# trvon/yams

Hardware: AMD Instinct MI355X
Metric: k-NN QPS + recall@k, 100M x 768 fp32 cosine top-100; ingest GB/s SHA-256+CDC (higher is better)
Workload: dtype i8 (MFMA filter, exact i32 accumulate) + f64 (exact re-score)

## Files before the change

yams_amd/csrc/scan_api.cpp:

```cpp
#include <chrono>
#include <algorithm>
#include <cmath>
#include <cstdio>
#include <cstdlib>
#include <cstring>
#include <vector>

#include "accel_ctx.h"
#include "scan_launch.h"

using namespace yams_accel;

namespace {

constexpr uint64_t kMfmaMinRows = 4096;
constexpr uint64_t kExactKeyBudget = 1ull << 31;
constexpr size_t kStatWords = 16;

uint32_t round_up(uint32_t v, uint32_t m) { return (v + m - 1) / m * m; }

ScanPlan make_plan(uint64_t n_rows, uint32_t dim, uint32_t nq, uint32_t k, bool bf16, int passes, bool l2_band, int depth = 0) {
    ScanPlan p;
    p.n_rows = n_rows; p.dim = dim; p.n_queries = nq;
    p.tile_rows = bf16 ? 256 : kTileRows;
// ... 457 lines not shown

yams_status_t run_filter(Batch& b, Filter& f, bool* done) {
    yams_accel_ctx* ctx = b.ctx; const yams_scan_corpus_t* corpus = b.io.corpus; hipStream_t st = b.st;
    const uint32_t nq = b.nq; const bool i8 = f.i8, bf16 = f.bf16;
    ScanLaunch& L = f.L; const ScanPlan& plan = L.plan;
    if (i8) L.dense = nullptr;
    else YA_TRY(ws_get(ctx, "dense", static_cast<size_t>(nq) * plan.sample_rows * 4, (void**)&L.dense));
    YA_TRY(ws_get(ctx, "gmax", static_cast<size_t>(nq) * plan.n_groups * 4, (void**)&L.gmax));
    YA_TRY(ws_get(ctx, "tau", static_cast<size_t>(nq) * 4, (void**)&f.d_tau));
    YA_TRY(ws_get(ctx, "list", static_cast<size_t>(nq) * plan.list_cap * 8, (void**)&f.d_list));
    const uint32_t gchunks = (plan.n_groups + kSelectCap - 1) / kSelectCap;
    YA_TRY(ws_get(ctx, "work32", static_cast<size_t>(2) * nq * std::max(1u, gchunks) * plan.tau_rank * 4, (void**)&f.d_work32));
    const uint32_t lchunks = (plan.list_cap + kSelectCap - 1) / kSelectCap, keep_max = kRescoreMax + 1;
    YA_TRY(ws_get(ctx, "work64", static_cast<size_t>(2) * nq * lchunks * keep_max * 8, (void**)&f.d_work64));
    L.tau = f.d_tau; L.tau_out = f.d_tau; L.list_count = b.d_lcount; L.list = f.d_list;
    if (i8) {
        L.i8_q_form = i8_takes_q_form(L, f.bf16_version);
        if (corpus->row_mask && corpus->row_mask_count) L.i8_mask_inflation = static_cast<double>(corpus->n_rows) / static_cast<double>(corpus->row_mask_count);
        const uint64_t regions = i8_log_regions(L);
        L.log_cap = i8_log_capacity(L);
        YA_TRY(ws_get(ctx, "i8_log_key", static_cast<size_t>(regions) * L.log_cap * i8_log_entry_bytes(L), (void**)&L.log_key));
        YA_TRY(ws_get(ctx, "i8_log_q", static_cast<size_t>(regions) * L.log_cap * 4, (void**)&L.log_q));
        const uint64_t sync_words = i8_sync_words(L);
        const size_t z_cnt = (static_cast<size_t>(regions) * 4 + 255) & ~size_t(255), z_over = (static_cast<size_t>(nq) * 4 + 255) & ~size_t(255);
        unsigned char* zeroed;
        YA_TRY(ws_get(ctx, "i8_zeroed", z_cnt + z_over + static_cast<size_t>(sync_words) * 4, (void**)&zeroed));
        XcdDealPrep deal{};
        uint64_t deal_words = 0;
        if (i8_xcd_deal_plan(L, &deal, &deal_words)) {
            YA_TRY(ws_get(ctx, "i8_xcd", static_cast<size_t>(deal_words) * 4, (void**)&L.i8_xcd));
// ... 19 lines not shown
                }
                k.forced = 1;
            }
#endif
        }
        YA_HIP(ctx, launch_prep_i8(st, b.d_qprep, nq, L.q_pad, b.dim, const_cast<int8_t*>(L.q_i8), const_cast<float*>(L.q_meta), L.i8_l2,
                                   reinterpret_cast<uint32_t*>(zeroed), (z_cnt + z_over) / 4 + sync_words, (corpus->i8_flags & YAMS_SCAN_I8_ROTATED) != 0, &deal));
        L.log_cnt = reinterpret_cast<uint32_t*>(zeroed);
        L.q_over = f.d_qover = reinterpret_cast<uint32_t*>(zeroed + z_cnt);
        if (sync_words) L.i8_sync = reinterpret_cast<uint32_t*>(zeroed + z_cnt + z_over);
    }
    { TimedRegion tr(ctx, "scan_sample");
      if (i8) YA_HIP(ctx, launch_scan_i8(st, L, 0, f.bf16_version));
      else if (bf16) YA_HIP(ctx, launch_scan_bf16(st, L, b.metric, 0, f.passes, f.bf16_version)); else YA_HIP(ctx, launch_scan_sample(st, L, b.metric));
      tr.end(); }
    if (b.retry) YA_HIP(ctx, hipMemcpyAsync(f.d_tau, b.retry->forced_tau, static_cast<size_t>(nq) * 4, hipMemcpyDeviceToDevice, st));
    else YA_HIP(ctx, launch_select_tau(st, L, f.d_work32));
    if (i8 && L.i8_l2) {
        YA_HIP(ctx, launch_i8_l2_thresholds(st, f.d_tau, L.q_meta, nq, L.q_pad, b.dim, b.d_l2_stats, const_cast<float*>(L.q_thr), const_cast<uint32_t*>(L.i8_q_bias)));
        YA_HIP(ctx, launch_i8_l2_rows(st, corpus->rows_nsq, corpus->rows_i8_meta, b.d_l2_nmin, corpus->n_rows, b.d_l2_stats, const_cast<float*>(L.i8_l2_meta),
                                      const_cast<uint8_t*>(L.i8_row_bias)));
    } else if (i8) YA_HIP(ctx, launch_i8_thresholds(st, f.d_tau, L.q_meta, nq, L.q_pad, const_cast<float*>(L.q_thr)));
    if (i8) YA_HIP(ctx, launch_i8_collect_sample(st, L)); else YA_HIP(ctx, launch_collect_sample(st, L));
    if (i8 && L.i8_l2) YA_HIP(ctx, launch_i8_l2_add_special(st, L, b.d_l2_special, b.l2_n_special));
    { GatedSweep gs(ctx, st);
      TimedRegion tr(ctx, "scan_filter");
      if (i8) YA_HIP(ctx, launch_scan_i8(st, L, 1, f.bf16_version));
      else if (bf16) YA_HIP(ctx, launch_scan_bf16(st, L, b.metric, 1, f.passes, f.bf16_version)); else YA_HIP(ctx, launch_scan_filter(st, L, b.metric));
      tr.end();
      gs.leave(); }
    if (i8) YA_HIP(ctx, launch_i8_log_gather(st, L));
#ifdef YAMS_ACCEL_MEASURE
    if (!(i8 && L.i8_sync)) {}
    else if (const char* dump = std::getenv("YAMS_ACCEL_DUMP_SYNC")) {
        std::vector<uint32_t> h(i8_sync_words(L));
        YA_HIP(ctx, hipMemcpyAsync(h.data(), L.i8_sync, h.size() * 4, hipMemcpyDeviceToHost, st));
        YA_HIP(ctx, hipStreamSynchronize(st));
// ... 458 lines not shown
```

yams_amd/csrc/scan_i8_kernel.hip:

```cpp
#include <climits>
#include <cstdlib>
#include <type_traits>

#include "lds_dma.h"
#include "scan_args.h"
#include "xcd_deal.h"

namespace yams_accel {

using i32x4v = __attribute__((ext_vector_type(4))) int;

constexpr int I8_ROWS = 256, I8_QUERIES = 256, I8_THREADS = 512;
constexpr int I8_SLAB = 64;
constexpr int I8_NST = 4;
constexpr int I8_A_BYTES = I8_ROWS * I8_SLAB;
constexpr int I8_B_BYTES = I8_QUERIES * I8_SLAB;
constexpr int I8_STAGE = I8_A_BYTES + I8_B_BYTES;
constexpr int I8_BLOCK_ROWS = 64;

__device__ __forceinline__ int i8_swz(int row) {
    const int j = (row >> 2) & 3;
    return (((j ^ (j >> 1)) & 1) << 1) | (j >> 1);
}

// ... 757 lines not shown
                asm volatile("s_waitcnt vmcnt(0)" ::: "memory");
                __builtin_amdgcn_sched_barrier(0);
            } else { qthr_wait(); thresholds(); }
            k_new = take_result();
            if (n_qt > 1 && more && pacing && pace_now) {
                asm volatile("" : "+v"(sib));
                uint32_t polls = 0;
                for (; polls < R_POLLS; ++polls) {
                    if (__builtin_amdgcn_ballot_w64(sib + R_WINDOW < k_new) == 0) break;
                    __builtin_amdgcn_s_sleep(8);
                    asm volatile("global_load_dword %0, %1, off sc0 sc1\n\ts_waitcnt vmcnt(0)" : "=v"(sib) : "v"(sync_sib) : "memory");
                }
                if (polls == R_POLLS) pacing = false;
            }
        } else if (SAMPLE) {
            asm volatile("s_waitcnt vmcnt(0)" ::: "memory");
            k_new = take_result();
            const uint32_t sel_c = 2u * u + (k_cur & 1u);
            if (sel_c < a.n_sel_tiles) {
                const float ninf = -__builtin_inff();
                const uint32_t gid = (sel_c * static_cast<uint32_t>(I8_ROWS) + static_cast<uint32_t>((wid & 3) * 64)) / 16u + static_cast<uint32_t>(lq);
#pragma unroll
                for (int cb = 0; cb < 8; ++cb) {
                    const uint32_t qi = q0 + static_cast<uint32_t>(cb * 16 + l15);
                    const float4 qm = reinterpret_cast<const float4*>(lds + R_ZS_THR)[cb * 16 + l15];
                    const float S = sb_cur * qm.x, K = fmaf(eb_cur, qm.y, qm.z);
                    float m = ninf;
#pragma unroll
                    for (int rb = 0; rb < 4; ++rb) {
                        const uint64_t rbase = strip + static_cast<uint32_t>(16 * rb + 4 * lq);
                        const uint32_t mw = a.row_mask ? mask_word(a.row_mask, rbase & ~31ull, a.n_rows) >> (rbase & 31u) : 0xfu;
#pragma unroll
                        for (int r = 0; r < 4; ++r) {
                            const float uu = fmaf(static_cast<float>(acc[rb][cb][r]), S, K);
                            m = fmaxf(m, (rbase + r < a.n_rows && ((mw >> r) & 1u)) ? uu : ninf);
                        }
                    }
                    if (qi < a.n_queries) a.gmax[static_cast<uint64_t>(qi) * a.n_groups + gid] = (m != m) ? 0xffffffffu : f2ord(m);
                }
            }
            sb = __uint_as_float(static_cast<uint32_t>(meta_n));
            eb = __uint_as_float(static_cast<uint32_t>(meta_n >> 32));
        } else {
            asm volatile("s_waitcnt vmcnt(0)" ::: "memory");
            k_new = take_result();
            int t = 0;
#pragma unroll
            for (int rb = 0; rb < 4; ++rb)
#pragma unroll
                for (int cb = 0; cb < 8; ++cb)
#pragma unroll
                    for (int r = 0; r < 4; ++r) t += acc[rb][cb][r];
            if (t == 123456789 && a.list_cap == 0xffffffffu) a.list_count[0] = 1;
// ... 108 lines not shown
        if (!i8_entry_score<L2>(keys[i], q, rows_meta, q_meta, q_thr, l2, row, u)) continue;
        const uint32_t pos = slot0[q - q0] + atomicAdd(&hist[q - q0], 1u);
        if (pos < list_cap) list[static_cast<uint64_t>(q) * list_cap + pos] = pack_key(u, row);
    }
}

#ifdef YAMS_ACCEL_MEASURE
#include "scan_i8q_gather.h"
#endif

__global__ __launch_bounds__(256) void i8_collect_sample_kernel(const uint32_t* gmax, uint32_t n_groups, uint32_t n_queries,
                                                                const int8_t* rows_i8, const float* rows_meta, const int8_t* q_i8,
                                                                const float* q_meta, uint32_t q_pad, uint32_t dim,
                                                                uint32_t stride, uint64_t n_rows, const uint32_t* row_mask,
                                                                const float* tau, uint32_t* list_count, uint64_t* list,
                                                                uint32_t list_cap, const float* l2_rows_nsq, float l2_eps) {
    const uint32_t q = blockIdx.y;
    const float t = tau[q];
    const uint32_t* gm = gmax + static_cast<uint64_t>(q) * n_groups;
    const uint32_t nchunk = dim / 16;
    const int lane = threadIdx.x & 63;
    const float4 qm = reinterpret_cast<const float4*>(q_meta)[q];
    const uint32_t wave0 = (blockIdx.x * blockDim.x + threadIdx.x) & ~63u, wstep = gridDim.x * blockDim.x;
    for (uint32_t g0 = wave0; g0 < n_groups; g0 += wstep) {
        const uint32_t gl = g0 + static_cast<uint32_t>(lane);
        const bool hot = gl < n_groups && !(ord2f(gm[gl]) < t);
        for (uint64_t hm = __builtin_amdgcn_ballot_w64(hot); hm; hm &= hm - 1) {
            const uint32_t g = g0 + static_cast<uint32_t>(__builtin_ctzll(hm));
            const int i = lane & 15;
            const uint64_t sidx = static_cast<uint64_t>(g >> 2) * 64 + 4 * (g & 3) + 16 * (i >> 2) + (i & 3);
            const uint64_t row = (sidx / I8_ROWS) * stride * I8_ROWS + (sidx % I8_ROWS);
            const bool ok = row < n_rows && (!row_mask || row_allowed(row_mask, row));
            const uint64_t rr = row < n_rows ? row : n_rows - 1;
            int dot = 0;
            for (uint32_t ch = static_cast<uint32_t>(lane >> 4); ch < nchunk; ch += 4) {
                const int4 xv = *reinterpret_cast<const int4*>(rows_i8 + i8_blocked_offset(rr, ch * 16, dim));
                const int4 qv = *reinterpret_cast<const int4*>(q_i8 + (static_cast<uint64_t>(ch >> 2) * q_pad + q) * 64 + (ch & 3u) * 16);
                dot = __builtin_amdgcn_sdot4(xv.x, qv.x, dot, false);
                dot = __builtin_amdgcn_sdot4(xv.y, qv.y, dot, false);
                dot = __builtin_amdgcn_sdot4(xv.z, qv.z, dot, false);
                dot = __builtin_amdgcn_sdot4(xv.w, qv.w, dot, false);
            }
            dot += __shfl_xor(dot, 16);
            dot += __shfl_xor(dot, 32);
            if (lane < 16 && ok) {
                const float2 bm = reinterpret_cast<const float2*>(rows_meta)[row / I8_BLOCK_ROWS];
                const float S = bm.x * qm.x, K = fmaf(bm.y, qm.y, qm.z);
                float u = fmaf(static_cast<float>(dot), S, K);
                bool unbounded = false;
                if (l2_rows_nsq) {
                    const float nsq = l2_rows_nsq[row];
                    unbounded = !norm_in_range(nsq);
                    u = i8_l2_bound(u, nsq, l2_eps);
                }
                if (!unbounded && !(u < t)) {
                    const uint32_t pos = atomicAdd(&list_count[q], 1u);
                    if (pos < list_cap) list[static_cast<uint64_t>(q) * list_cap + pos] = pack_key(u, static_cast<uint32_t>(row));
                }
            }
        }
    }
}

__device__ inline uint32_t rot_sign(uint32_t i, uint32_t salt) {
    uint32_t v = i * 2654435761u + salt * 0x9E3779B9u;
    v ^= v >> 15; v *= 2246822519u; v ^= v >> 13; v *= 3266489917u; v ^= v >> 16;
    return v << 31;
}
__device__ inline void wave_lds_fence() {
    __builtin_amdgcn_fence(__ATOMIC_ACQ_REL, "wavefront");
    __builtin_amdgcn_wave_barrier();
}
template <int EPL>
__device__ inline void wave_fwht(float* w, int lane, uint32_t g0, uint32_t sign_salt, float scale) {
    float v[EPL];
// ... 288 lines not shown
    if (threadIdx.x == 0) {
        const float fd = static_cast<float>(dim);
        const float up = 1.0f + (fd + 16.f) * 5.9604645e-8f;
        q_meta[4 * q + 0] = t;
        q_meta[4 * q + 1] = ok ? sqrtf(csum) * up : 0.f;
        const float unit = raw ? (rot_p ? (sqrtf(csum) + sqrtf(red[0])) * up * 1.00001f : sqrtf(csum) * up) : 1.0f;
        q_meta[4 * q + 2] = ok ? sqrtf(red[0]) * up + ((fd + 32.f) * 5.9604645e-8f + 1e-6f + (rot_p ? 1e-5f : 0.f)) * unit : 0.f;
        q_meta[4 * q + 3] = 0.f;
    }
}

__global__ void i8_query_thresholds_kernel(const float* tau, const float* q_meta, uint32_t nq, uint32_t q_pad, float* q_thr) {
    const uint32_t q = blockIdx.x * blockDim.x + threadIdx.x;
    if (q >= q_pad) return;
    float A = __builtin_inff(), B = 0.f;
    if (q < nq) {
        const float t = q_meta[4 * q], c = q_meta[4 * q + 1], f = q_meta[4 * q + 2], ta = tau[q];
        if (ta != ta) A = -__builtin_inff();
        else {
            A = (ta - f) / t;
            A -= fabsf(A) * 1.9073486e-6f;
        }
        B = (c / t) * (1.0f + 1.9073486e-6f);
    }
    q_thr[2 * q] = A;
    q_thr[2 * q + 1] = B;
}

constexpr int L2S_WAVES = 16;
constexpr uint32_t I8_L2_MAX_SPECIAL = 64;
__global__ __launch_bounds__(L2S_WAVES * 64) void i8_l2_norm_stats_kernel(const float* rows_nsq, const float* rows_meta, uint64_t n_rows,
                                                                         uint64_t n_blocks, float* nmin_out, uint32_t* stats,
                                                                         uint32_t* special) {
    __shared__ uint32_t red[L2S_WAVES][5];
    const int lane = threadIdx.x & 63, wid = threadIdx.x >> 6;
    float qlo = __builtin_inff(), qhi = 0.f, sp = 0.f, em = 0.f;
    constexpr int NB = 4;
    const uint64_t step = static_cast<uint64_t>(gridDim.x) * L2S_WAVES;
    for (uint64_t blk0 = static_cast<uint64_t>(blockIdx.x) * L2S_WAVES + wid; blk0 < n_blocks; blk0 += step * NB) {
// ... 278 lines not shown
bool i8_takes_q_form(const ScanLaunch&, int) { return false; }
uint32_t i8_log_entry_bytes(const ScanLaunch&) { return 8u; }
#endif

uint64_t i8_log_regions(const ScanLaunch& L) {
    const ResidentPlan r = i8_resident_plan(L);
    if (r.use && L.i8_q_form) return static_cast<uint64_t>(r.n_streams) * r.n_qt * 4u;
    if (r.use) return static_cast<uint64_t>(r.n_streams) * r.n_qt * 8u;
    return static_cast<uint64_t>((2u * L.plan.n_filter_tiles + 7) / 8) * L.plan.n_qtiles * 8u * 4u;
}

hipError_t launch_i8_collect_sample(hipStream_t st, const ScanLaunch& L) {
    if (L.plan.sample_rows == 0 || L.plan.n_groups == 0) return hipSuccess;
    uint32_t gx = (L.plan.n_groups + 255) / 256;
    if (gx > 64) gx = 64;
#ifdef YAMS_ACCEL_MEASURE
    if (const char* e = std::getenv("YAMS_ACCEL_COLLECT_GX")) { const uint32_t v = static_cast<uint32_t>(std::atoi(e)); if (v >= 1 && v < gx) gx = v; }
#endif
    hipLaunchKernelGGL(i8_collect_sample_kernel, dim3(gx, L.plan.n_queries), dim3(256), 0, st, L.gmax, L.plan.n_groups,
                       L.plan.n_queries, L.rows_i8, L.rows_i8_meta, L.q_i8, L.q_meta, L.q_pad, L.plan.dim, L.plan.sample_stride,
                       L.plan.n_rows, L.row_mask, L.tau, L.list_count, L.list, L.plan.list_cap,
                       L.i8_l2 ? L.rows_nsq : nullptr, L.l2_eps);
    return hipGetLastError();
}

bool i8_xcd_deal_plan(const ScanLaunch& L, XcdDealPrep* p, uint64_t* table_words) {
    const ResidentPlan r = i8_resident_plan(L);
    if (!r.use) return false;
    p->n_units_filter = r.n_units;
    p->n_units_sample = (L.plan.n_sample_tiles + 1u) / 2u;
    p->streams_x = r.n_streams / XCD_DEAL_XCDS;
    p->n_qt = r.n_qt;
    *table_words = XCD_TABLE_TICKS + static_cast<uint64_t>(r.n_streams) * r.n_qt * XCD_TICKS_PER_WG;
    return true;
}

uint64_t i8_sync_words(const ScanLaunch& L) {
// ... 181 lines not shown
```

yams_amd/csrc/scan_kernels.hip:

```cpp
#include <algorithm>

#include "common.h"
#include "scan_args.h"

namespace yams_accel {

using f32x16 = __attribute__((ext_vector_type(16))) float;

constexpr int LDP = kSlabK + 4;
constexpr int STAGE_FLOATS = (kTileRows + kTileQueries) * LDP;
constexpr int SCAN_THREADS = 256;


template <int MODE, int METRIC>
__global__ __launch_bounds__(SCAN_THREADS, 2) void scan_tiles_kernel(ScanArgs a) {
    __shared__ __attribute__((aligned(16))) float lds[2 * STAGE_FLOATS];

    const uint32_t bid = blockIdx.x;
    const uint32_t xcd = bid & 7u;
    const uint32_t w = bid >> 3;
    const uint32_t qt = w % a.n_qtiles;
    const uint32_t sel = (w / a.n_qtiles) * 8u + xcd;
    if (sel >= a.n_sel_tiles) return;
    uint32_t tile;
// ... 388 lines not shown
    K* dst = out + static_cast<uint64_t>(qslot) * out_stride + static_cast<uint64_t>(blockIdx.x) * keep;
    if (c0 >= n) {
        for (uint32_t i = threadIdx.x; i < keep; i += 256) dst[i] = K(0);
        return;
    }
    const uint64_t left = n - c0;
    const uint64_t end = left < static_cast<uint64_t>(CAP) ? n : c0 + CAP;
    if (left <= 256) topk_block_sorted<K, 1>(src, c0, end, dst, keep, s);
    else if (left <= 512) topk_block_sorted<K, 2>(src, c0, end, dst, keep, s);
    else if (left <= 1024) topk_block_sorted<K, 4>(src, c0, end, dst, keep, s);
    else if (left <= 2048) topk_block_sorted<K, 8>(src, c0, end, dst, keep, s);
    else topk_block_sorted<K, 16>(src, c0, end, dst, keep, s);
}

constexpr int TAU_LIST = 2048;
__global__ __launch_bounds__(256) void tau_select_kernel(const uint32_t* gmax, uint32_t n_groups,
                                                         uint32_t rank, float* tau, const float* rows_meta, uint64_t n_blocks,
                                                         const float* q_meta, uint32_t rank2, uint32_t max_groups, float e_scale) {
    __shared__ uint32_t hist[2048];
    __shared__ uint32_t s_prefix, s_rank, s_count, s_v1, s_v2, s_va;
    __shared__ float s_red[4];
    const uint32_t q = blockIdx.x;
    const uint32_t* keys = gmax + static_cast<uint64_t>(q) * n_groups;
    if (n_groups < rank) {
        if (threadIdx.x == 0) tau[q] = -__builtin_inff();
        return;
    }
    if (rank >= 1 && rank <= 256) {
        const float e_mine = rows_meta != nullptr && n_blocks ? rows_meta[2 * ((n_blocks - 1) * threadIdx.x / 255) + 1] : 0.f;
        uint32_t mine = 0;
        for (uint32_t i = threadIdx.x; i < n_groups; i += 256) { const uint32_t k = keys[i]; mine = k > mine ? k : mine; }
        hist[threadIdx.x] = mine;
        if (threadIdx.x == 0) { s_count = 0; s_v1 = 0; s_v2 = 0; s_va = 0; }
        __syncthreads();
        uint32_t above = 0, at_or_above = 0;
        for (int j = 0; j < 256; ++j) { const uint32_t o = hist[j]; above += o > mine; at_or_above += o >= mine; }
        if (above < rank && rank <= at_or_above) s_prefix = mine;
        __syncthreads();
        const uint32_t L = s_prefix;
        __syncthreads();
        bool overflow = false;
        if (mine >= L)
            for (uint32_t i = threadIdx.x; i < n_groups; i += 256) {
                const uint32_t k = keys[i];
                if (k >= L) {
                    const uint32_t pos = atomicAdd(&s_count, 1u);
                    if (pos < TAU_LIST) hist[pos] = k; else overflow = true;
                }
            }
        if (!__syncthreads_or(overflow)) {
            const uint32_t c = s_count;
            if (max_groups > n_groups / 64) max_groups = n_groups / 64;
            const bool aware = rows_meta != nullptr && rank2 >= 5 && rank2 < rank && max_groups >= rank2;
            const uint32_t rank_a = rank2 - 4;
            for (uint32_t i = threadIdx.x; i < c; i += 256) {
                const uint32_t k = hist[i];
                uint32_t gt = 0, ge = 0;
                for (uint32_t j = 0; j < c; ++j) { const uint32_t o = hist[j]; gt += o > k; ge += o >= k; }
                if (gt < rank && rank <= ge) {
                    if (aware) s_v1 = k; else tau[q] = k ? ord2f(k) : -__builtin_inff();
                }
                if (aware && gt < rank2 && rank2 <= ge) s_v2 = k;
                if (aware && gt < rank_a && rank_a <= ge) s_va = k;
            }
            if (!aware) return;
            float e = e_mine;
#pragma unroll
            for (int d = 32; d >= 1; d >>= 1) e = fmaxf(e, __shfl_xor(e, d));
            if ((threadIdx.x & 63) == 0) s_red[threadIdx.x >> 6] = e;
            __syncthreads();
            const uint32_t v1 = s_v1, v2 = s_v2, va = s_va;
            float t_out = v1 ? ord2f(v1) : -__builtin_inff();
            bool want = false;
            float tp = 0.f;
            if (v1 && v2 && va) {
                e = fmaxf(fmaxf(s_red[0], s_red[1]), fmaxf(s_red[2], s_red[3]));
                const float4 qm = reinterpret_cast<const float4*>(q_meta)[q];
                const float E = fmaf(e, qm.y, qm.z) * e_scale;
                tp = ord2f(v2) - 2.0f * E;
                want = ord2f(va) - t_out < E && tp < t_out;
            }
            if (want) {
                const uint32_t lb = __syncthreads_count(mine != 0 && !(ord2f(mine) < tp));
                uint32_t n_reach = 0xffffffffu;
                if (lb <= max_groups) {
                    uint32_t cnt = 0;
                    for (uint32_t i = threadIdx.x; i < n_groups; i += 256) { const uint32_t k = keys[i]; cnt += k != 0 && !(ord2f(k) < tp); }
#pragma unroll
                    for (int d = 32; d >= 1; d >>= 1) cnt += __shfl_xor(cnt, d);
                    __syncthreads();
                    if ((threadIdx.x & 63) == 0) s_red[threadIdx.x >> 6] = __uint_as_float(cnt);
                    __syncthreads();
                    n_reach = __float_as_uint(s_red[0]) + __float_as_uint(s_red[1]) + __float_as_uint(s_red[2]) + __float_as_uint(s_red[3]);
                }
                if (n_reach <= max_groups) t_out = tp;
            }
            if (threadIdx.x == 0) tau[q] = t_out;
            return;
        }
        __syncthreads();
    }
    if (threadIdx.x == 0) { s_prefix = 0; s_rank = rank; }
    const int shifts[3] = {21, 10, 0};
    const int widths[3] = {11, 11, 10};
    for (int p = 0; p < 3; ++p) {
        const int shift = shifts[p], bins = 1 << widths[p];
        for (int i = threadIdx.x; i < 2048; i += 256) hist[i] = 0;
        __syncthreads();
        const uint32_t prefix = s_prefix;
        const int hi_shift = shift + widths[p];
        for (uint32_t i = threadIdx.x; i < n_groups; i += 256) {
            const uint32_t k = keys[i];
// ... 15 lines not shown
            const uint32_t r = s_rank;
            if (r > excl && r <= incl) {
                uint32_t above = excl;
                for (int j = 0; j < per; ++j) {
                    const int b = bins - 1 - (lane * per + j);
                    const uint32_t c = hist[b];
                    if (r <= above + c) { s_prefix = (prefix << widths[p]) | static_cast<uint32_t>(b); s_rank = r - above; break; }
                    above += c;
                }
            }
        }
        __syncthreads();
    }
    if (threadIdx.x == 0) {
        const uint32_t key = s_prefix;
        tau[q] = key ? ord2f(key) : -__builtin_inff();
    }
}

__global__ __launch_bounds__(256) void collect_sample_kernel(const float* dense, const uint32_t* gmax,
                                                             uint32_t n_groups, uint32_t n_queries,
                                                             uint64_t sample_rows, uint32_t tile_rows,
                                                             uint32_t stride,
                                                             uint64_t n_rows, const float* tau,
                                                             uint32_t* list_count, uint64_t* list,
                                                             uint32_t list_cap, int layout16) {
    const uint32_t q = blockIdx.y;
    const float t = tau[q];
    const uint32_t* gm = gmax + static_cast<uint64_t>(q) * n_groups;
    for (uint32_t g = blockIdx.x * blockDim.x + threadIdx.x; g < n_groups; g += gridDim.x * blockDim.x) {
        const float m = ord2f(gm[g]);
// ... 715 lines not shown
        cur = dst; cur_counts = nullptr; cur_stride = dst_stride; cur_n = chunks * keep;
        cur_qmap = nullptr;
        count_clip = 0xffffffffu;
        which ^= 1;
        if (chunks == 1) break;
    }
    *result = cur;
    *result_stride = cur_stride;
    return hipSuccess;
}

hipError_t launch_select_tau(hipStream_t st, const ScanLaunch& L, uint32_t* ) {
    const uint32_t nq = L.plan.n_queries;
    if (nq == 0) return hipSuccess;
    hipLaunchKernelGGL(tau_select_kernel, dim3(nq), dim3(256), 0, st, L.gmax, L.plan.n_groups,
                       L.plan.tau_rank, L.tau_out, L.tau_rows_meta, L.tau_n_blocks, L.q_meta, L.tau_rank2, L.tau_max_groups, L.tau_e_scale);
    LAUNCH_CHECK();
    return hipSuccess;
}

hipError_t launch_collect_sample(hipStream_t st, const ScanLaunch& L) {
    if (L.plan.sample_rows == 0 || L.plan.n_groups == 0) return hipSuccess;
    uint32_t gx = (L.plan.n_groups + 255) / 256;
    if (gx > 256) gx = 256;
    hipLaunchKernelGGL(collect_sample_kernel, dim3(gx, L.plan.n_queries), dim3(256), 0, st, L.dense,
                       L.gmax, L.plan.n_groups, L.plan.n_queries, L.plan.sample_rows, L.plan.tile_rows,
                       L.plan.sample_stride, L.plan.n_rows, L.tau, L.list_count, L.list, L.plan.list_cap,
                       L.sample_layout);
    LAUNCH_CHECK();
    return hipSuccess;
}
// ... 297 lines not shown
```

yams_amd/csrc/scan_launch.h:

```cpp
#pragma once
#include "common.h"
#include "xcd_deal.h"

namespace yams_accel {

struct ScanLaunch {
    ScanPlan plan;
    const float* rows = nullptr;
    const uint16_t* rows_bf16 = nullptr;
    const float* rows_nsq = nullptr;
    const int8_t* rows_i8 = nullptr;
    const float* rows_i8_meta = nullptr;
    const int8_t* q_i8 = nullptr;
    const float* q_meta = nullptr;
    const float* q_thr = nullptr;
    uint64_t* log_key = nullptr; uint32_t* log_q = nullptr; uint32_t* log_cnt = nullptr; uint32_t log_cap = 0;
    uint32_t* q_over = nullptr;
    uint32_t* i8_sync = nullptr;
    uint32_t* i8_xcd = nullptr;
    bool i8_l2 = false;
    const float* i8_l2_meta = nullptr;
    const uint8_t* i8_row_bias = nullptr;
    const uint32_t* i8_q_bias = nullptr;
    float l2_eps = 0.f;
    bool i8_sample_small_grid = false;
    int i8_form = 0;
    bool i8_q_form = false;
    double i8_mask_inflation = 1.0;
    int sample_layout = 0;
    const uint32_t* row_mask = nullptr;
    const float* qprep = nullptr;
    const uint16_t* q_hi = nullptr;
    const uint16_t* q_lo = nullptr;
    uint32_t q_pad = 0;
    float* dense = nullptr;
    uint32_t* gmax = nullptr;
    const float* tau = nullptr;
    float* tau_out = nullptr;
    const float* tau_rows_meta = nullptr; uint64_t tau_n_blocks = 0; uint32_t tau_rank2 = 0, tau_max_groups = 0; float tau_e_scale = 1.0f;
    uint32_t* list_count = nullptr;
    uint64_t* list = nullptr;
    const float* qnorm_up = nullptr;
    float err_coef = 0.f;
};

struct RescoreLaunch {
    const float* rows; uint64_t n_rows; uint32_t dim;
    const float* queries; const double* qnorm;
    const uint32_t* tie_rank; const uint32_t* rank_row; int64_t row_base;
    uint32_t stripe_rows, n_stripes, stripe_index;
    const uint64_t* cand; uint64_t cand_stride; uint32_t n_cand;
    const float* tau; const uint32_t* list_count; uint32_t list_cap; uint32_t all_rows_listed;
    const uint32_t* qmap; uint32_t n_slots;
    uint32_t k; float threshold; uint32_t flags; double err_bound;
// ... 116 lines not shown
```

Measured before the change: 16990.

## Chain tau select into thresholds and hot-group list; precompute sample group keys

The tau selection kernel now also writes the i8 query thresholds, which removes the separate threshold launch on the non-L2 path. It also records the indices of groups at or above tau in a small per-query hot list. The collect-sample kernel reads that list and scores only those groups, skipping the full gmax scan, and its grid is capped lower when the list is present. Separately, the sample-pass group max keys are computed before the vmcnt wait, using an integer-max fast path, so they overlap with outstanding loads. The cost is more LDS and branching in tau_select, plus a fallback to the full scan when the list overflows or a key is zero.

```diff
diff --git a/yams_amd/csrc/sample_chain.h b/yams_amd/csrc/sample_chain.h
--- /dev/null
+++ b/yams_amd/csrc/sample_chain.h
@@ -0,0 +1,39 @@
+#pragma once
+#include "contract_rules.h"
+
+namespace yams_accel {
+
+YAMS_RULE bool sample_max_int_ok(float S, float K) {
+    uint32_t sb, kb;
+    __builtin_memcpy(&sb, &S, 4);
+    __builtin_memcpy(&kb, &K, 4);
+    return sb < 0x7f800000u && (kb & 0x7fffffffu) < 0x7f800000u && kb != 0x80000000u;
+}
+
+YAMS_RULE uint32_t sample_group_key_int(int acc_max, bool any, float S, float K) {
+    return any ? f2ord(fmaf(static_cast<float>(acc_max), S, K)) : f2ord(-__builtin_inff());
+}
+
+YAMS_RULE uint32_t sample_group_key_rows(const int* acc, uint32_t live, float S, float K) {
+    float m = -__builtin_inff();
+    for (int l = 0; l < 16; ++l) {
+        const float uu = fmaf(static_cast<float>(acc[l]), S, K);
+        m = fmaxf(m, ((live >> l) & 1u) ? uu : -__builtin_inff());
+    }
+    return (m != m) ? 0xffffffffu : f2ord(m);
+}
+
+YAMS_RULE void i8_threshold_halves(float ta, float t, float c, float f, float& A, float& B) {
+    if (ta != ta) A = -__builtin_inff();
+    else {
+        A = (ta - f) / t;
+        A -= fabsf(A) * 1.9073486e-6f;
+    }
+    B = (c / t) * (1.0f + 1.9073486e-6f);
+}
+
+constexpr uint32_t HOT_STRIDE = 128, HOT_CAP = HOT_STRIDE - 1, HOT_SCAN = 0xffffffffu;
+
+YAMS_RULE bool hot_threshold_listable(float t) { return t == t && t != 0.0f; }
+
+}
diff --git a/yams_amd/csrc/scan_api.cpp b/yams_amd/csrc/scan_api.cpp
--- a/yams_amd/csrc/scan_api.cpp
+++ b/yams_amd/csrc/scan_api.cpp
@@ -7,6 +7,7 @@
 #include <vector>
 
 #include "accel_ctx.h"
+#include "sample_chain.h"
 #include "scan_launch.h"
 
 using namespace yams_accel;
@@ -495,6 +496,8 @@
     const uint32_t lchunks = (plan.list_cap + kSelectCap - 1) / kSelectCap, keep_max = kRescoreMax + 1;
     YA_TRY(ws_get(ctx, "work64", static_cast<size_t>(2) * nq * lchunks * keep_max * 8, (void**)&f.d_work64));
     L.tau = f.d_tau; L.tau_out = f.d_tau; L.list_count = b.d_lcount; L.list = f.d_list;
+    uint32_t* d_hot = nullptr;
+    if (i8) YA_TRY(ws_get(ctx, "i8_hot", static_cast<size_t>(nq) * HOT_STRIDE * 4, (void**)&d_hot));
     if (i8) {
         L.i8_q_form = i8_takes_q_form(L, f.bf16_version);
         if (corpus->row_mask && corpus->row_mask_count) L.i8_mask_inflation = static_cast<double>(corpus->n_rows) / static_cast<double>(corpus->row_mask_count);
@@ -544,13 +547,16 @@
       if (i8) YA_HIP(ctx, launch_scan_i8(st, L, 0, f.bf16_version));
       else if (bf16) YA_HIP(ctx, launch_scan_bf16(st, L, b.metric, 0, f.passes, f.bf16_version)); else YA_HIP(ctx, launch_scan_sample(st, L, b.metric));
       tr.end(); }
+    const bool tau_chain = i8 && !L.i8_l2 && !b.retry;
+    L.tau_q_thr = tau_chain ? const_cast<float*>(L.q_thr) : nullptr;
+    L.tau_hot = tau_chain ? d_hot : nullptr;
     if (b.retry) YA_HIP(ctx, hipMemcpyAsync(f.d_tau, b.retry->forced_tau, static_cast<size_t>(nq) * 4, hipMemcpyDeviceToDevice, st));
     else YA_HIP(ctx, launch_select_tau(st, L, f.d_work32));
     if (i8 && L.i8_l2) {
         YA_HIP(ctx, launch_i8_l2_thresholds(st, f.d_tau, L.q_meta, nq, L.q_pad, b.dim, b.d_l2_stats, const_cast<float*>(L.q_thr), const_cast<uint32_t*>(L.i8_q_bias)));
         YA_HIP(ctx, launch_i8_l2_rows(st, corpus->rows_nsq, corpus->rows_i8_meta, b.d_l2_nmin, corpus->n_rows, b.d_l2_stats, const_cast<float*>(L.i8_l2_meta),
                                       const_cast<uint8_t*>(L.i8_row_bias)));
-    } else if (i8) YA_HIP(ctx, launch_i8_thresholds(st, f.d_tau, L.q_meta, nq, L.q_pad, const_cast<float*>(L.q_thr)));
+    } else if (i8 && !tau_chain) YA_HIP(ctx, launch_i8_thresholds(st, f.d_tau, L.q_meta, nq, L.q_pad, const_cast<float*>(L.q_thr)));
     if (i8) YA_HIP(ctx, launch_i8_collect_sample(st, L)); else YA_HIP(ctx, launch_collect_sample(st, L));
     if (i8 && L.i8_l2) YA_HIP(ctx, launch_i8_l2_add_special(st, L, b.d_l2_special, b.l2_n_special));
     { GatedSweep gs(ctx, st);
diff --git a/yams_amd/csrc/scan_i8_kernel.hip b/yams_amd/csrc/scan_i8_kernel.hip
--- a/yams_amd/csrc/scan_i8_kernel.hip
+++ b/yams_amd/csrc/scan_i8_kernel.hip
@@ -5,6 +5,7 @@
 #include "lds_dma.h"
 #include "scan_args.h"
 #include "xcd_deal.h"
+#include "sample_chain.h"
 
 namespace yams_accel {
 
@@ -795,29 +796,64 @@
                 if (polls == R_POLLS) pacing = false;
             }
         } else if (SAMPLE) {
+            const uint32_t sel_c = 2u * u + (k_cur & 1u);
+            const bool emit = sel_c < a.n_sel_tiles;
+            uint32_t gkey[8];
+            if (emit) {
+                uint32_t live = 0;
+#pragma unroll
+                for (int rb = 0; rb < 4; ++rb) {
+                    const uint64_t rbase = strip + static_cast<uint32_t>(16 * rb + 4 * lq);
+                    const uint32_t mw = a.row_mask ? mask_word(a.row_mask, rbase & ~31ull, a.n_rows) >> (rbase & 31u) : 0xfu;
+#pragma unroll
+                    for (int r = 0; r < 4; ++r) live |= (rbase + r < a.n_rows && ((mw >> r) & 1u)) ? 1u << (4 * rb + r) : 0u;
+                }
+                const bool all_live = __builtin_amdgcn_ballot_w64(live != 0xffffu) == 0;
+#pragma unroll
+                for (int cb = 0; cb < 8; ++cb) {
+                    const float4 qm = reinterpret_cast<const float4*>(lds + R_ZS_THR)[cb * 16 + l15];
+                    const float S = sb_cur * qm.x, K = fmaf(eb_cur, qm.y, qm.z);
+                    if (__builtin_amdgcn_ballot_w64(!sample_max_int_ok(S, K)) == 0) {
+                        int mx = INT_MIN;
+                        if (all_live) {
+#pragma unroll
+                            for (int rb = 0; rb < 4; ++rb)
+#pragma unroll
+                                for (int r = 0; r < 4; ++r) mx = acc[rb][cb][r] > mx ? acc[rb][cb][r] : mx;
+                        } else {
+#pragma unroll
+                            for (int rb = 0; rb < 4; ++rb)
+#pragma unroll
+                                for (int r = 0; r < 4; ++r) {
+                                    const int v = ((live >> (4 * rb + r)) & 1u) ? acc[rb][cb][r] : INT_MIN;
+                                    mx = v > mx ? v : mx;
+                                }
+                        }
+                        gkey[cb] = sample_group_key_int(mx, live != 0u, S, K);
+                    } else {
+                        const float ninf = -__builtin_inff();
+                        float m = ninf;
+#pragma unroll
+                        for (int rb = 0; rb < 4; ++rb)
+#pragma unroll
+                            for (int r = 0; r < 4; ++r) {
+                                const float uu = fmaf(static_cast<float>(acc[rb][cb][r]), S, K);
+                                m = fmaxf(m, ((live >> (4 * rb + r)) & 1u) ? uu : ninf);
+                            }
+                        gkey[cb] = (m != m) ? 0xffffffffu : f2ord(m);
+                    }
+                }
+            }
+            __builtin_amdgcn_sched_barrier(0);
             asm volatile("s_waitcnt vmcnt(0)" ::: "memory");
+            __builtin_amdgcn_sched_barrier(0);
             k_new = take_result();
-            const uint32_t sel_c = 2u * u + (k_cur & 1u);
-            if (sel_c < a.n_sel_tiles) {
-                const float ninf = -__builtin_inff();
+            if (emit) {
                 const uint32_t gid = (sel_c * static_cast<uint32_t>(I8_ROWS) + static_cast<uint32_t>((wid & 3) * 64)) / 16u + static_cast<uint32_t>(lq);
 #pragma unroll
                 for (int cb = 0; cb < 8; ++cb) {
                     const uint32_t qi = q0 + static_cast<uint32_t>(cb * 16 + l15);
-                    const float4 qm = reinterpret_cast<const float4*>(lds + R_ZS_THR)[cb * 16 + l15];
-                    const float S = sb_cur * qm.x, K = fmaf(eb_cur, qm.y, qm.z);
-                    float m = ninf;
-#pragma unroll
-                    for (int rb = 0; rb < 4; ++rb) {
-                        const uint64_t rbase = strip + static_cast<uint32_t>(16 * rb + 4 * lq);
-                        const uint32_t mw = a.row_mask ? mask_word(a.row_mask, rbase & ~31ull, a.n_rows) >> (rbase & 31u) : 0xfu;
-#pragma unroll
-                        for (int r = 0; r < 4; ++r) {
-                            const float uu = fmaf(static_cast<float>(acc[rb][cb][r]), S, K);
-                            m = fmaxf(m, (rbase + r < a.n_rows && ((mw >> r) & 1u)) ? uu : ninf);
-                        }
-                    }
-                    if (qi < a.n_queries) a.gmax[static_cast<uint64_t>(qi) * a.n_groups + gid] = (m != m) ? 0xffffffffu : f2ord(m);
+                    if (qi < a.n_queries) a.gmax[static_cast<uint64_t>(qi) * a.n_groups + gid] = gkey[cb];
                 }
             }
             sb = __uint_as_float(static_cast<uint32_t>(meta_n));
@@ -956,51 +992,60 @@
                                                                 const float* q_meta, uint32_t q_pad, uint32_t dim,
                                                                 uint32_t stride, uint64_t n_rows, const uint32_t* row_mask,
                                                                 const float* tau, uint32_t* list_count, uint64_t* list,
-                                                                uint32_t list_cap, const float* l2_rows_nsq, float l2_eps) {
+                                                                uint32_t list_cap, const float* l2_rows_nsq, float l2_eps,
+                                                                const uint32_t* hot_list) {
     const uint32_t q = blockIdx.y;
     const float t = tau[q];
     const uint32_t* gm = gmax + static_cast<uint64_t>(q) * n_groups;
     const uint32_t nchunk = dim / 16;
     const int lane = threadIdx.x & 63;
     const float4 qm = reinterpret_cast<const float4*>(q_meta)[q];
+    auto score_group = [&](uint32_t g) {
+        const int i = lane & 15;
+        const uint64_t sidx = static_cast<uint64_t>(g >> 2) * 64 + 4 * (g & 3) + 16 * (i >> 2) + (i & 3);
+        const uint64_t row = (sidx / I8_ROWS) * stride * I8_ROWS + (sidx % I8_ROWS);
+        const bool ok = row < n_rows && (!row_mask || row_allowed(row_mask, row));
+        const uint64_t rr = row < n_rows ? row : n_rows - 1;
+        int dot = 0;
+        for (uint32_t ch = static_cast<uint32_t>(lane >> 4); ch < nchunk; ch += 4) {
+            const int4 xv = *reinterpret_cast<const int4*>(rows_i8 + i8_blocked_offset(rr, ch * 16, dim));
+            const int4 qv = *reinterpret_cast<const int4*>(q_i8 + (static_cast<uint64_t>(ch >> 2) * q_pad + q) * 64 + (ch & 3u) * 16);
+            dot = __builtin_amdgcn_sdot4(xv.x, qv.x, dot, false);
+            dot = __builtin_amdgcn_sdot4(xv.y, qv.y, dot, false);
+            dot = __builtin_amdgcn_sdot4(xv.z, qv.z, dot, false);
+            dot = __builtin_amdgcn_sdot4(xv.w, qv.w, dot, false);
+        }
+        dot += __shfl_xor(dot, 16);
+        dot += __shfl_xor(dot, 32);
+        if (lane < 16 && ok) {
+            const float2 bm = reinterpret_cast<const float2*>(rows_meta)[row / I8_BLOCK_ROWS];
+            const float S = bm.x * qm.x, K = fmaf(bm.y, qm.y, qm.z);
+            float u = fmaf(static_cast<float>(dot), S, K);
+            bool unbounded = false;
+            if (l2_rows_nsq) {
+                const float nsq = l2_rows_nsq[row];
+                unbounded = !norm_in_range(nsq);
+                u = i8_l2_bound(u, nsq, l2_eps);
+            }
+            if (!unbounded && !(u < t)) {
+                const uint32_t pos = atomicAdd(&list_count[q], 1u);
+                if (pos < list_cap) list[static_cast<uint64_t>(q) * list_cap + pos] = pack_key(u, static_cast<uint32_t>(row));
+            }
+        }
+    };
     const uint32_t wave0 = (blockIdx.x * blockDim.x + threadIdx.x) & ~63u, wstep = gridDim.x * blockDim.x;
+    const uint32_t n_hot = hot_list ? hot_list[static_cast<uint64_t>(q) * HOT_STRIDE] : HOT_SCAN;
+    if (n_hot != HOT_SCAN) {
+        for (uint32_t j = wave0 / 64u; j < n_hot && j < HOT_CAP; j += wstep / 64u) {
+            const uint32_t g = hot_list[static_cast<uint64_t>(q) * HOT_STRIDE + 1u + j];
+            if (g < n_groups) score_group(g);
+        }
+        return;
+    }
     for (uint32_t g0 = wave0; g0 < n_groups; g0 += wstep) {
         const uint32_t gl = g0 + static_cast<uint32_t>(lane);
         const bool hot = gl < n_groups && !(ord2f(gm[gl]) < t);
-        for (uint64_t hm = __builtin_amdgcn_ballot_w64(hot); hm; hm &= hm - 1) {
-            const uint32_t g = g0 + static_cast<uint32_t>(__builtin_ctzll(hm));
-            const int i = lane & 15;
-            const uint64_t sidx = static_cast<uint64_t>(g >> 2) * 64 + 4 * (g & 3) + 16 * (i >> 2) + (i & 3);
-            const uint64_t row = (sidx / I8_ROWS) * stride * I8_ROWS + (sidx % I8_ROWS);
-            const bool ok = row < n_rows && (!row_mask || row_allowed(row_mask, row));
-            const uint64_t rr = row < n_rows ? row : n_rows - 1;
-            int dot = 0;
-            for (uint32_t ch = static_cast<uint32_t>(lane >> 4); ch < nchunk; ch += 4) {
-                const int4 xv = *reinterpret_cast<const int4*>(rows_i8 + i8_blocked_offset(rr, ch * 16, dim));
-                const int4 qv = *reinterpret_cast<const int4*>(q_i8 + (static_cast<uint64_t>(ch >> 2) * q_pad + q) * 64 + (ch & 3u) * 16);
-                dot = __builtin_amdgcn_sdot4(xv.x, qv.x, dot, false);
-                dot = __builtin_amdgcn_sdot4(xv.y, qv.y, dot, false);
-                dot = __builtin_amdgcn_sdot4(xv.z, qv.z, dot, false);
-                dot = __builtin_amdgcn_sdot4(xv.w, qv.w, dot, false);
-            }
-            dot += __shfl_xor(dot, 16);
-            dot += __shfl_xor(dot, 32);
-            if (lane < 16 && ok) {
-                const float2 bm = reinterpret_cast<const float2*>(rows_meta)[row / I8_BLOCK_ROWS];
-                const float S = bm.x * qm.x, K = fmaf(bm.y, qm.y, qm.z);
-                float u = fmaf(static_cast<float>(dot), S, K);
-                bool unbounded = false;
-                if (l2_rows_nsq) {
-                    const float nsq = l2_rows_nsq[row];
-                    unbounded = !norm_in_range(nsq);
-                    u = i8_l2_bound(u, nsq, l2_eps);
-                }
-                if (!unbounded && !(u < t)) {
-                    const uint32_t pos = atomicAdd(&list_count[q], 1u);
-                    if (pos < list_cap) list[static_cast<uint64_t>(q) * list_cap + pos] = pack_key(u, static_cast<uint32_t>(row));
-                }
-            }
-        }
+        for (uint64_t hm = __builtin_amdgcn_ballot_w64(hot); hm; hm &= hm - 1) score_group(g0 + static_cast<uint32_t>(__builtin_ctzll(hm)));
     }
 }
 
@@ -1319,15 +1364,7 @@
     const uint32_t q = blockIdx.x * blockDim.x + threadIdx.x;
     if (q >= q_pad) return;
     float A = __builtin_inff(), B = 0.f;
-    if (q < nq) {
-        const float t = q_meta[4 * q], c = q_meta[4 * q + 1], f = q_meta[4 * q + 2], ta = tau[q];
-        if (ta != ta) A = -__builtin_inff();
-        else {
-            A = (ta - f) / t;
-            A -= fabsf(A) * 1.9073486e-6f;
-        }
-        B = (c / t) * (1.0f + 1.9073486e-6f);
-    }
+    if (q < nq) i8_threshold_halves(tau[q], q_meta[4 * q], q_meta[4 * q + 1], q_meta[4 * q + 2], A, B);
     q_thr[2 * q] = A;
     q_thr[2 * q + 1] = B;
 }
@@ -1636,13 +1673,14 @@
     if (L.plan.sample_rows == 0 || L.plan.n_groups == 0) return hipSuccess;
     uint32_t gx = (L.plan.n_groups + 255) / 256;
     if (gx > 64) gx = 64;
+    if (L.tau_hot && gx > 8) gx = 8;
 #ifdef YAMS_ACCEL_MEASURE
     if (const char* e = std::getenv("YAMS_ACCEL_COLLECT_GX")) { const uint32_t v = static_cast<uint32_t>(std::atoi(e)); if (v >= 1 && v < gx) gx = v; }
 #endif
     hipLaunchKernelGGL(i8_collect_sample_kernel, dim3(gx, L.plan.n_queries), dim3(256), 0, st, L.gmax, L.plan.n_groups,
                        L.plan.n_queries, L.rows_i8, L.rows_i8_meta, L.q_i8, L.q_meta, L.q_pad, L.plan.dim, L.plan.sample_stride,
                        L.plan.n_rows, L.row_mask, L.tau, L.list_count, L.list, L.plan.list_cap,
-                       L.i8_l2 ? L.rows_nsq : nullptr, L.l2_eps);
+                       L.i8_l2 ? L.rows_nsq : nullptr, L.l2_eps, L.tau_hot);
     return hipGetLastError();
 }
 
diff --git a/yams_amd/csrc/scan_kernels.hip b/yams_amd/csrc/scan_kernels.hip
--- a/yams_amd/csrc/scan_kernels.hip
+++ b/yams_amd/csrc/scan_kernels.hip
@@ -2,6 +2,7 @@
 
 #include "common.h"
 #include "scan_args.h"
+#include "sample_chain.h"
 
 namespace yams_accel {
 
@@ -426,25 +427,56 @@
 }
 
 constexpr int TAU_LIST = 2048;
+template <typename F>
+__device__ __forceinline__ void tau_keys_strided(const uint32_t* keys, uint32_t n, F&& f) {
+    for (uint32_t i = threadIdx.x; i < n; i += 16u * 256u) {
+        uint32_t k[16];
+#pragma unroll
+        for (int u = 0; u < 16; ++u) k[u] = i + static_cast<uint32_t>(u) * 256u < n ? keys[i + static_cast<uint32_t>(u) * 256u] : 0u;
+#pragma unroll
+        for (int u = 0; u < 16; ++u)
+            if (i + static_cast<uint32_t>(u) * 256u < n) f(i + static_cast<uint32_t>(u) * 256u, k[u]);
+    }
+}
+
+struct TauChain { float* q_thr; uint32_t n_queries, q_pad; uint32_t* hot; };
+
 __global__ __launch_bounds__(256) void tau_select_kernel(const uint32_t* gmax, uint32_t n_groups,
                                                          uint32_t rank, float* tau, const float* rows_meta, uint64_t n_blocks,
-                                                         const float* q_meta, uint32_t rank2, uint32_t max_groups, float e_scale) {
+                                                         const float* q_meta, uint32_t rank2, uint32_t max_groups, float e_scale,
+                                                         TauChain ch) {
     __shared__ uint32_t hist[2048];
-    __shared__ uint32_t s_prefix, s_rank, s_count, s_v1, s_v2, s_va;
+    __shared__ uint32_t hid[TAU_LIST];
+    __shared__ uint32_t s_hot[HOT_CAP];
+    __shared__ uint32_t s_prefix, s_rank, s_count, s_v1, s_v2, s_va, s_hn;
     __shared__ float s_red[4];
     const uint32_t q = blockIdx.x;
     const uint32_t* keys = gmax + static_cast<uint64_t>(q) * n_groups;
+    if (ch.q_thr && q == 0)
+        for (uint32_t i = ch.n_queries + threadIdx.x; i < ch.q_pad; i += 256) { ch.q_thr[2 * i] = __builtin_inff(); ch.q_thr[2 * i + 1] = 0.f; }
+    auto store_tau = [&](float t_out) {
+        tau[q] = t_out;
+        if (ch.q_thr) {
+            const float4 qm = reinterpret_cast<const float4*>(q_meta)[q];
+            float A, B;
+            i8_threshold_halves(t_out, qm.x, qm.y, qm.z, A, B);
+            ch.q_thr[2 * q] = A;
+            ch.q_thr[2 * q + 1] = B;
+        }
+    };
+    uint32_t* const hot_q = ch.hot ? ch.hot + static_cast<uint64_t>(q) * HOT_STRIDE : nullptr;
     if (n_groups < rank) {
-        if (threadIdx.x == 0) tau[q] = -__builtin_inff();
+        if (threadIdx.x == 0) { store_tau(-__builtin_inff()); if (hot_q) hot_q[0] = HOT_SCAN; }
         return;
     }
     if (rank >= 1 && rank <= 256) {
         const float e_mine = rows_meta != nullptr && n_blocks ? rows_meta[2 * ((n_blocks - 1) * threadIdx.x / 255) + 1] : 0.f;
         uint32_t mine = 0;
-        for (uint32_t i = threadIdx.x; i < n_groups; i += 256) { const uint32_t k = keys[i]; mine = k > mine ? k : mine; }
+        bool zero = false;
+        tau_keys_strided(keys, n_groups, [&](uint32_t, uint32_t k) { mine = k > mine ? k : mine; zero |= k == 0u; });
         hist[threadIdx.x] = mine;
-        if (threadIdx.x == 0) { s_count = 0; s_v1 = 0; s_v2 = 0; s_va = 0; }
-        __syncthreads();
+        if (threadIdx.x == 0) { s_count = 0; s_v1 = 0; s_v2 = 0; s_va = 0; s_hn = 0; }
+        const bool any_zero = __syncthreads_or(zero);
         uint32_t above = 0, at_or_above = 0;
         for (int j = 0; j < 256; ++j) { const uint32_t o = hist[j]; above += o > mine; at_or_above += o >= mine; }
         if (above < rank && rank <= at_or_above) s_prefix = mine;
@@ -453,13 +485,12 @@
         __syncthreads();
         bool overflow = false;
         if (mine >= L)
-            for (uint32_t i = threadIdx.x; i < n_groups; i += 256) {
-                const uint32_t k = keys[i];
+            tau_keys_strided(keys, n_groups, [&](uint32_t i, uint32_t k) {
                 if (k >= L) {
                     const uint32_t pos = atomicAdd(&s_count, 1u);
-                    if (pos < TAU_LIST) hist[pos] = k; else overflow = true;
-                }
-            }
+                    if (pos < TAU_LIST) { hist[pos] = k; hid[pos] = i; } else overflow = true;
+                }
+            });
         if (!__syncthreads_or(overflow)) {
             const uint32_t c = s_count;
             if (max_groups > n_groups / 64) max_groups = n_groups / 64;
@@ -469,45 +500,73 @@
                 const uint32_t k = hist[i];
                 uint32_t gt = 0, ge = 0;
                 for (uint32_t j = 0; j < c; ++j) { const uint32_t o = hist[j]; gt += o > k; ge += o >= k; }
-                if (gt < rank && rank <= ge) {
-                    if (aware) s_v1 = k; else tau[q] = k ? ord2f(k) : -__builtin_inff();
-                }
+                if (gt < rank && rank <= ge) s_v1 = k;
                 if (aware && gt < rank2 && rank2 <= ge) s_v2 = k;
                 if (aware && gt < rank_a && rank_a <= ge) s_va = k;
             }
-            if (!aware) return;
-            float e = e_mine;
-#pragma unroll
-            for (int d = 32; d >= 1; d >>= 1) e = fmaxf(e, __shfl_xor(e, d));
-            if ((threadIdx.x & 63) == 0) s_red[threadIdx.x >> 6] = e;
             __syncthreads();
-            const uint32_t v1 = s_v1, v2 = s_v2, va = s_va;
+            const uint32_t v1 = s_v1;
             float t_out = v1 ? ord2f(v1) : -__builtin_inff();
-            bool want = false;
-            float tp = 0.f;
-            if (v1 && v2 && va) {
-                e = fmaxf(fmaxf(s_red[0], s_red[1]), fmaxf(s_red[2], s_red[3]));
-                const float4 qm = reinterpret_cast<const float4*>(q_meta)[q];
-                const float E = fmaf(e, qm.y, qm.z) * e_scale;
-                tp = ord2f(v2) - 2.0f * E;
-                want = ord2f(va) - t_out < E && tp < t_out;
-            }
-            if (want) {
-                const uint32_t lb = __syncthreads_count(mine != 0 && !(ord2f(mine) < tp));
-                uint32_t n_reach = 0xffffffffu;
-                if (lb <= max_groups) {
-                    uint32_t cnt = 0;
-                    for (uint32_t i = threadIdx.x; i < n_groups; i += 256) { const uint32_t k = keys[i]; cnt += k != 0 && !(ord2f(k) < tp); }
-#pragma unroll
-                    for (int d = 32; d >= 1; d >>= 1) cnt += __shfl_xor(cnt, d);
-                    __syncthreads();
-                    if ((threadIdx.x & 63) == 0) s_red[threadIdx.x >> 6] = __uint_as_float(cnt);
-                    __syncthreads();
-                    n_reach = __float_as_uint(s_red[0]) + __float_as_uint(s_red[1]) + __float_as_uint(s_red[2]) + __float_as_uint(s_red[3]);
-                }
-                if (n_reach <= max_groups) t_out = tp;
-            }
-            if (threadIdx.x == 0) tau[q] = t_out;
+            bool deeper = false;
+            if (aware) {
+                float e = e_mine;
+#pragma unroll
+                for (int d = 32; d >= 1; d >>= 1) e = fmaxf(e, __shfl_xor(e, d));
+                if ((threadIdx.x & 63) == 0) s_red[threadIdx.x >> 6] = e;
+                __syncthreads();
+                const uint32_t v2 = s_v2, va = s_va;
+                bool want = false;
+                float tp = 0.f;
+                if (v1 && v2 && va) {
+                    e = fmaxf(fmaxf(s_red[0], s_red[1]), fmaxf(s_red[2], s_red[3]));
+                    const float4 qm = reinterpret_cast<const float4*>(q_meta)[q];
+                    const float E = fmaf(e, qm.y, qm.z) * e_scale;
+                    tp = ord2f(v2) - 2.0f * E;
+                    want = ord2f(va) - t_out < E && tp < t_out;
+                }
+                if (want) {
+                    const uint32_t lb = __syncthreads_count(mine != 0 && !(ord2f(mine) < tp));
+                    uint32_t n_reach = 0xffffffffu;
+                    if (lb <= max_groups) {
+                        uint32_t cnt = 0;
+                        tau_keys_strided(keys, n_groups, [&](uint32_t i, uint32_t k) {
+                            if (k != 0 && !(ord2f(k) < tp)) {
+                                ++cnt;
+                                if (hot_q) { const uint32_t pos = atomicAdd(&s_hn, 1u); if (pos < HOT_CAP) s_hot[pos] = i; }
+                            }
+                        });
+#pragma unroll
+                        for (int d = 32; d >= 1; d >>= 1) cnt += __shfl_xor(cnt, d);
+                        __syncthreads();
+                        if ((threadIdx.x & 63) == 0) s_red[threadIdx.x >> 6] = __uint_as_float(cnt);
+                        __syncthreads();
+                        n_reach = __float_as_uint(s_red[0]) + __float_as_uint(s_red[1]) + __float_as_uint(s_red[2]) + __float_as_uint(s_red[3]);
+                    }
+                    if (n_reach <= max_groups) { t_out = tp; deeper = true; }
+                }
+            }
+            if (threadIdx.x == 0) store_tau(t_out);
+            if (!hot_q) return;
+            if (any_zero || !hot_threshold_listable(t_out)) {
+                if (threadIdx.x == 0) hot_q[0] = HOT_SCAN;
+                return;
+            }
+            if (deeper) {
+                const uint32_t n = s_hn;
+                if (n <= HOT_CAP)
+                    for (uint32_t i = threadIdx.x; i < n; i += 256) hot_q[1 + i] = s_hot[i];
+                if (threadIdx.x == 0) hot_q[0] = n <= HOT_CAP ? n : HOT_SCAN;
+                return;
+            }
+            if (threadIdx.x == 0) s_hn = 0;
+            __syncthreads();
+            for (uint32_t i = threadIdx.x; i < c; i += 256)
+                if (!(ord2f(hist[i]) < t_out)) {
+                    const uint32_t pos = atomicAdd(&s_hn, 1u);
+                    if (pos < HOT_CAP) hot_q[1 + pos] = hid[i];
+                }
+            __syncthreads();
+            if (threadIdx.x == 0) hot_q[0] = s_hn <= HOT_CAP ? s_hn : HOT_SCAN;
             return;
         }
         __syncthreads();
@@ -553,7 +612,8 @@
     }
     if (threadIdx.x == 0) {
         const uint32_t key = s_prefix;
-        tau[q] = key ? ord2f(key) : -__builtin_inff();
+        store_tau(key ? ord2f(key) : -__builtin_inff());
+        if (hot_q) hot_q[0] = HOT_SCAN;
     }
 }
 
@@ -1299,7 +1359,8 @@
     const uint32_t nq = L.plan.n_queries;
     if (nq == 0) return hipSuccess;
     hipLaunchKernelGGL(tau_select_kernel, dim3(nq), dim3(256), 0, st, L.gmax, L.plan.n_groups,
-                       L.plan.tau_rank, L.tau_out, L.tau_rows_meta, L.tau_n_blocks, L.q_meta, L.tau_rank2, L.tau_max_groups, L.tau_e_scale);
+                       L.plan.tau_rank, L.tau_out, L.tau_rows_meta, L.tau_n_blocks, L.q_meta, L.tau_rank2, L.tau_max_groups, L.tau_e_scale,
+                       TauChain{L.tau_q_thr, nq, L.q_pad, L.tau_hot});
     LAUNCH_CHECK();
     return hipSuccess;
 }
diff --git a/yams_amd/csrc/scan_launch.h b/yams_amd/csrc/scan_launch.h
--- a/yams_amd/csrc/scan_launch.h
+++ b/yams_amd/csrc/scan_launch.h
@@ -38,6 +38,7 @@
     const float* tau = nullptr;
     float* tau_out = nullptr;
     const float* tau_rows_meta = nullptr; uint64_t tau_n_blocks = 0; uint32_t tau_rank2 = 0, tau_max_groups = 0; float tau_e_scale = 1.0f;
+    float* tau_q_thr = nullptr; uint32_t* tau_hot = nullptr;
     uint32_t* list_count = nullptr;
     uint64_t* list = nullptr;
     const float* qnorm_up = nullptr;
```

Result: no change. 17070 (median of 6 runs) (+0.5%).
